# sabarim/STEm-Seg

Measured on AMD Instinct MI355X. Metric: clips/sec (T=8, 480p) embed+cluster, higher is better.
Workload: dtype f16x3: fp32 emulated from 2 fp16 terms per operand (22-bit operand significands; fp32 has 24), power-of-two operand scaling, 3 fp16 MFMA products per fp32 product, fp32 accumulate; |activation| >= 2.6e5 -> non-finite, flagged on the device, clip re-run in bf16x6

## Files before the change

stem-seg_amd/build.py:

```python
#!/usr/bin/env python3
import hashlib
import json
import os
import re
import subprocess
import sys
from concurrent.futures import ThreadPoolExecutor

HERE = os.path.dirname(os.path.abspath(__file__))
CSRC = os.path.join(HERE, "csrc")
LIBDIR = os.path.join(HERE, "stemseg_amd", "lib")
OBJDIR = os.path.join(CSRC, "build")
LIB = os.path.join(LIBDIR, "libstemseg_hip.so")
ARCH = "gfx950"
FLAGS = ["--offload-arch=" + ARCH, "-O3", "-std=c++17", "-fPIC", "-fno-gpu-rdc", "-Wall", "-Wno-unused-function"]
FLAGS += ["-Xclang", "-target-feature", "-Xclang", "-packed-fp32-ops"]
FLAGS += ["-save-temps=obj"]
PACKED_FP32 = re.compile(r"^\s+(v_pk_(?:fma|mul|add)_f32)\b")


def _sources():
    return sorted(f for f in os.listdir(CSRC) if f.endswith(".hip"))


def _digest():
    h = hashlib.sha256()
    h.update(" ".join(FLAGS).encode())
    for f in sorted(os.listdir(CSRC)) + [os.path.join("..", "..", "include", "stemseg_hip.h")]:
        p = os.path.join(CSRC, f)
        if os.path.isfile(p) and (f.endswith((".hip", ".h"))):
            h.update(f.encode())
            h.update(open(p, "rb").read())
    return h.hexdigest()


def isa_report():
    out = {}
    for src in _sources():
        path = os.path.join(OBJDIR, src.replace(".hip", "") + "-hip-amdgcn-amd-amdhsa-gfx950.s")
        kernels, by_kernel, cur = 0, {}, None
        if os.path.exists(path):
            for line in open(path, errors="replace"):
                m = re.match(r"^(_Z\w+|\w+):\s*(;.*)?$", line)
                if m and not line.startswith("."):
                    cur = m.group(1)
                if ".amdhsa_kernel " in line:
                    kernels += 1
                m = PACKED_FP32.match(line)
                if m and cur:
                    by_kernel[cur] = by_kernel.get(cur, 0) + 1
        out[src] = {"kernels": kernels, "packed_fp32_valu_instructions": sum(by_kernel.values()), "kernels_with_packed_fp32": len(by_kernel),
                    "assembly_found": os.path.exists(path)}
    return {"arch": ARCH, "no_packed_fp32_flag": True, "sources": out}


def build(force=False, verbose=True):
    os.makedirs(LIBDIR, exist_ok=True)
    os.makedirs(OBJDIR, exist_ok=True)
    stamp = os.path.join(OBJDIR, "libstemseg_hip.stamp")
    dig = _digest()
    if not force and os.path.exists(LIB) and os.path.exists(stamp) and open(stamp).read().strip() == dig:
        if verbose:
            print("[build] %s is up to date" % os.path.relpath(LIB, os.path.dirname(HERE)))
        return LIB
    hipcc = os.environ.get("HIPCC", "/opt/rocm/bin/hipcc")
    if not os.path.exists(hipcc):
        hipcc = "hipcc"

    def compile_one(src):
        obj = os.path.join(OBJDIR, src.replace(".hip", ".o"))
        cmd = [hipcc] + FLAGS + ["-c", os.path.join(CSRC, src), "-o", obj]
        r = subprocess.run(cmd, capture_output=True, text=True)
        if r.returncode != 0:
            raise RuntimeError("hipcc failed on %s:\n%s\n%s" % (src, r.stdout, r.stderr))
        err = "\n".join(l for l in r.stderr.splitlines() if "is not a recognized feature for this target" not in l).strip()
        if verbose and err:
            print(err)
        stem = os.path.join(OBJDIR, src.replace(".hip", ""))
        for ext in ("-hip-amdgcn-amd-amdhsa-gfx950.hipi", "-hip-amdgcn-amd-amdhsa-gfx950.bc", "-host-x86_64-unknown-linux-gnu.hipi",
                    "-host-x86_64-unknown-linux-gnu.bc", "-host-x86_64-unknown-linux-gnu.s"):
            if os.path.exists(stem + ext):
                os.remove(stem + ext)
        return obj

    with ThreadPoolExecutor(max_workers=min(8, os.cpu_count() or 2)) as ex:
# ... 21 lines not shown
```

stem-seg_amd/csrc/bottleneck_fused.hip:

```cpp
#include "common.h"
#include "split_operand.h"

namespace stemseg {

typedef float f32x16 __attribute__((ext_vector_type(16)));
typedef _Float16 f16x8 __attribute__((ext_vector_type(8)));
typedef unsigned int u32x4 __attribute__((ext_vector_type(4)));

struct FusedTailParams {
    const unsigned int* x16;
    const char* w3;
    const float* b3;
    const float* res;
    float* y;
    const char* w1;
    const float* b1;
    float* z;
    int64_t z_cs, z_ts, z_ys;
    int dec_H, dec_W;
    int V;
    const float* xs;
    const char* wd;
    const float* bd;
    float* xsub;
// ... 370 lines not shown

template <int MID_>
struct FusedTail16Cfg {
    static constexpr int MID = MID_, COUT = 4 * MID_, CT = 128;
    static constexpr int NW = 8, NTHREADS = 512, P = 16 * NW;
    static constexpr int NC3 = MID / 32, NCT = COUT / CT;
    static constexpr int NT3 = CT / 16, NT1 = MID / 16;
    static constexpr int SC = 2;
    static constexpr int NS = NC3 / SC, NU = CT / 32;
    static constexpr int W3_CHUNK = 8 * CT * 16;
    static constexpr int W3_BYTES = SC * W3_CHUNK;
    static constexpr int W1_BYTES = 8 * MID * 16;
    static constexpr int TAB_BYTES = 2 * CT * 4;
    static constexpr int LDS_BYTES = 2 * W3_BYTES + 2 * W1_BYTES + 2 * TAB_BYTES;
    static_assert(NC3 % SC == 0 && W3_BYTES % (1024 * NW) == 0 && W1_BYTES % (1024 * NW) == 0 && TAB_BYTES == 1024, "whole DMA pieces per wave");
    static_assert(W3_CHUNK == FT_WL.slab_bytes(CT, FT_WL.CK) && W1_BYTES == FT_WL.slab_bytes(MID, FT_WL.CK), "tile byte sizes follow the packed-weight layout");
    static_assert(LDS_BYTES <= 160 * 1024 && 2 * MID * 4 <= W3_BYTES, "LDS");
};

template <class C>
__global__ __launch_bounds__(C::NTHREADS, 2) void fused_tail16_kernel(const FusedTailParams p) {
#pragma clang fp contract(off)
    __shared__ __attribute__((aligned(1024))) char smem[C::LDS_BYTES];
    char* const w3buf = smem;
    char* const w1buf = smem + 2 * C::W3_BYTES;
    char* const tabbuf = smem + 2 * C::W3_BYTES + 2 * C::W1_BYTES;

    const int tid = threadIdx.x, lane = tid & 63;
    const int wave = __builtin_amdgcn_readfirstlane(tid >> 6);
    const int n = lane & 15, kb = lane >> 4;
    const int pos = blockIdx.x * C::P + wave * 16 + n;
    const bool pos_ok = pos < p.V;
    const int pos_c = min(pos, p.V - 1);
    const int64_t V = p.V;
    const unsigned int lane_off = (unsigned int)(((int64_t)(4 * kb) * V + pos_c) * 4);
    auto opaque = [](unsigned int v) __attribute__((always_inline)) { asm volatile("" : "+v"(v)); return v; };
    typedef const __attribute__((address_space(1))) void* gptr_t;
    typedef __attribute__((address_space(3))) void* lptr_t;
    const float* inv3 = reinterpret_cast<const float*>(p.w3 + FT_WL.inv_offset(C::COUT, C::MID));
    const float* inv1 = reinterpret_cast<const float*>(p.w1 + FT_WL.inv_offset(C::MID, C::COUT));

    auto dma_w3 = [&](const int j, const int st, const int buf) __attribute__((always_inline)) {
        constexpr int PER_ROW = C::CT * 16 / 1024, PER_CHUNK = C::W3_CHUNK / 1024;
#pragma unroll
        for (int k = 0; k < C::W3_BYTES / 1024 / C::NW; ++k) {
            const int idx = wave + k * C::NW, sc = idx / PER_CHUNK, r = idx % PER_CHUNK, row = r / PER_ROW, part = r % PER_ROW;
            const char* src = p.w3 + ((int64_t)(st * C::SC + sc) * 8 + row) * (C::COUT * 16) + (int64_t)j * (C::CT * 16) + part * 1024 + (size_t)(opaque((unsigned int)lane) * 16u);
            __builtin_amdgcn_global_load_lds((gptr_t)src, (lptr_t)(w3buf + buf * C::W3_BYTES + idx * 1024), 16, 0, 0);
        }
    };
    auto dma_w1 = [&](const int cc, const int buf) __attribute__((always_inline)) {
#pragma unroll
        for (int k = 0; k < C::W1_BYTES / 1024 / C::NW; ++k) {
            const int idx = wave + k * C::NW;
            const char* src = p.w1 + (int64_t)cc * C::W1_BYTES + (int64_t)idx * 1024 + (size_t)(opaque((unsigned int)lane) * 16u);
            __builtin_amdgcn_global_load_lds((gptr_t)src, (lptr_t)(w1buf + buf * C::W1_BYTES + idx * 1024), 16, 0, 0);
        }
    };
    auto dma_tab = [&](const int j) __attribute__((always_inline)) {
        if (wave == 0) {
            const unsigned int l = opaque((unsigned int)lane);
            const float* src = (l < 32 ? inv3 : p.b3 - C::CT) + (int64_t)j * C::CT + (size_t)(l * 4u);
            __builtin_amdgcn_global_load_lds((gptr_t)src, (lptr_t)(tabbuf + (j & 1) * C::TAB_BYTES), 16, 0, 0);
        }
    };
    auto dma_tail_tab = [&]() __attribute__((always_inline)) {
        constexpr int PIECES = (2 * C::MID + 255) / 256;
        if (wave < PIECES) {
            const unsigned int f0 = (unsigned int)wave * 256u + opaque((unsigned int)lane) * 4u;
            if (f0 < 2u * C::MID) {
                const float* src = (f0 < (unsigned int)C::MID ? inv1 : p.b1 - C::MID) + (size_t)f0;
                __builtin_amdgcn_global_load_lds((gptr_t)src, (lptr_t)(w3buf + wave * 1024), 16, 0, 0);
            }
        }
    };
    auto stage_sync = [&]() __attribute__((always_inline)) {
        __builtin_amdgcn_s_waitcnt(0x0f70);
        __syncthreads();
    };
    auto load_identity = [&](const int co_first, float (&rres)[8]) __attribute__((always_inline)) {
// ... 1 lines not shown
        for (int i = 0; i < 8; ++i)
            rres[i] = *reinterpret_cast<const float*>(reinterpret_cast<const char*>(p.res + (int64_t)(co_first + 16 * (i >> 2) + (i & 3)) * V) + (size_t)lane_off);
    };
    const f16x8 k2048 = {(_Float16)(1.0f / F16X3_LO_SCALE), (_Float16)(1.0f / F16X3_LO_SCALE), (_Float16)(1.0f / F16X3_LO_SCALE), (_Float16)(1.0f / F16X3_LO_SCALE),
                         (_Float16)(1.0f / F16X3_LO_SCALE), (_Float16)(1.0f / F16X3_LO_SCALE), (_Float16)(1.0f / F16X3_LO_SCALE), (_Float16)(1.0f / F16X3_LO_SCALE)};
    auto mma3x2 = [&](f32x4& c0, f32x4& c1, const f16x8 a0_hi, const f16x8 a0_lo, const f16x8 a1_hi, const f16x8 a1_lo, const f16x8 b_hi, const f16x8 b_lo)
        __attribute__((always_inline)) {
        const f16x8 a0_his = a0_hi * k2048, a1_his = a1_hi * k2048;
        c0 = __builtin_amdgcn_mfma_f32_16x16x32_f16(a0_lo, b_hi, c0, 0, 0, 0);
        c1 = __builtin_amdgcn_mfma_f32_16x16x32_f16(a1_lo, b_hi, c1, 0, 0, 0);
        c0 = __builtin_amdgcn_mfma_f32_16x16x32_f16(a0_his, b_lo, c0, 0, 0, 0);
        c1 = __builtin_amdgcn_mfma_f32_16x16x32_f16(a1_his, b_lo, c1, 0, 0, 0);
        c0 = __builtin_amdgcn_mfma_f32_16x16x32_f16(a0_hi, b_hi, c0, 0, 0, 0);
        c1 = __builtin_amdgcn_mfma_f32_16x16x32_f16(a1_hi, b_hi, c1, 0, 0, 0);
    };

    dma_w3(0, 0, 0);
    f16x8 xh[C::NC3], xl[C::NC3];
    {
        const char* xs = reinterpret_cast<const char*>(p.x16) + (size_t)((unsigned int)pos_c * 16u);
#pragma unroll
        for (int s = 0; s < C::NC3; ++s) {
            xh[s] = *reinterpret_cast<const f16x8*>(xs + ((int64_t)(4 * s + kb)) * V * 16);
            xl[s] = *reinterpret_cast<const f16x8*>(xs + ((int64_t)(C::MID / 8 + 4 * s + kb)) * V * 16);
        }
    }
    f32x4 acc1[C::NT1];
#pragma unroll
    for (int m = 0; m < C::NT1; ++m) acc1[m] = f32x4{0.f, 0.f, 0.f, 0.f};
    stage_sync();
    int sb = 0, eb = 0;
#pragma unroll 1
    for (int j = 0; j < C::NCT; ++j) {
        f32x4 acc3[C::NT3];
#pragma unroll
        for (int t = 0; t < C::NT3; ++t) acc3[t] = f32x4{0.f, 0.f, 0.f, 0.f};
        const int co_j = j * C::CT;
        float rres[8];
#pragma unroll
        for (int st = 0; st < C::NS; ++st) {
            if (st + 1 < C::NS) dma_w3(j, st + 1, sb ^ 1);
            else { dma_w1(j * C::NU, eb); dma_tab(j); load_identity(co_j, rres); }
            const char* wb = w3buf + sb * C::W3_BYTES + (((kb >> 1) * 2 * 2 + (kb & 1)) * C::CT + n) * 16;
            constexpr int NSTEP = C::SC * C::NT3 / 2;
            f16x8 a_hi[2][2], a_lo[2][2];
            auto ld_a = [&](const int i, const int k) __attribute__((always_inline)) {
                const int sc = (2 * i) / C::NT3, t = (2 * i) % C::NT3;
#pragma unroll
                for (int e = 0; e < 2; ++e) {
                    a_hi[k][e] = *reinterpret_cast<const f16x8*>(wb + sc * C::W3_CHUNK + (0 * 2 * C::CT + (t + e) * 16) * 16);
                    a_lo[k][e] = *reinterpret_cast<const f16x8*>(wb + sc * C::W3_CHUNK + (1 * 2 * C::CT + (t + e) * 16) * 16);
                }
            };
            ld_a(0, 0);
#pragma unroll
            for (int i = 0; i < NSTEP; ++i) {
                if (i + 1 < NSTEP) ld_a(i + 1, (i + 1) & 1);
                __builtin_amdgcn_sched_barrier(0);
                const int t = (2 * i) % C::NT3, ch = st * C::SC + (2 * i) / C::NT3;
                mma3x2(acc3[t], acc3[t + 1], a_hi[i & 1][0], a_lo[i & 1][0], a_hi[i & 1][1], a_lo[i & 1][1], xh[ch], xl[ch]);
                __builtin_amdgcn_sched_barrier(0);
            }
            stage_sync();
            sb ^= 1;
        }
        const float* tab = reinterpret_cast<const float*>(tabbuf + (j & 1) * C::TAB_BYTES);
// ... 31 lines not shown
                    auto s16 = __builtin_amdgcn_permlane16_swap(s32[0], s32[1], false, false);
                    bw[pl][i] = s16[0];
                    bw[pl][2 + i] = s16[1];
                }
            const u32x4 bh = {bw[0][0], bw[0][1], bw[0][2], bw[0][3]}, bl = {bw[1][0], bw[1][1], bw[1][2], bw[1][3]};
            const f16x8 b_hi = __builtin_bit_cast(f16x8, bh), b_lo = __builtin_bit_cast(f16x8, bl);
            __builtin_amdgcn_sched_barrier(0);
            if (u + 1 < C::NU) { dma_w1(j * C::NU + u + 1, eb ^ 1); load_identity(co_j + 32 * (u + 1), rres); }
            else if (j + 1 < C::NCT) dma_w3(j + 1, 0, sb);
            else dma_tail_tab();
            __builtin_amdgcn_sched_barrier(0);
            const char* w1b = w1buf + eb * C::W1_BYTES + (((kb >> 1) * 2 * 2 + (kb & 1)) * C::MID + n) * 16;
            f16x8 a_hi[1][2], a_lo[1][2];
            auto ld_a1 = [&](const int i, const int k) __attribute__((always_inline)) {
#pragma unroll
                for (int e = 0; e < 2; ++e) {
                    a_hi[k][e] = *reinterpret_cast<const f16x8*>(w1b + (0 * 2 * C::MID + (2 * i + e) * 16) * 16);
                    a_lo[k][e] = *reinterpret_cast<const f16x8*>(w1b + (1 * 2 * C::MID + (2 * i + e) * 16) * 16);
                }
            };
#pragma unroll
            for (int i = 0; i < C::NT1 / 2; ++i) {
                ld_a1(i, 0);
                __builtin_amdgcn_sched_barrier(0);
                mma3x2(acc1[2 * i], acc1[2 * i + 1], a_hi[0][0], a_lo[0][0], a_hi[0][1], a_lo[0][1], b_hi, b_lo);
                __builtin_amdgcn_sched_barrier(0);
            }
            stage_sync();
            eb ^= 1;
        }
    }
    if (pos_ok) {
        const int hwp = p.dec_H * p.dec_W;
        const int t2 = pos / hwp, r2 = pos - t2 * hwp, y2 = r2 / p.dec_W, x2 = r2 - y2 * p.dec_W;
        const unsigned int z_off = (unsigned int)(((int64_t)(4 * kb) * p.z_cs + (int64_t)t2 * p.z_ts + (int64_t)y2 * p.z_ys + x2) * 4);
        const float* ttab = reinterpret_cast<const float*>(w3buf);
#pragma unroll
        for (int m1 = 0; m1 < C::NT1; ++m1) {
            const int co4 = m1 * 16 + 4 * kb;
            const float4 sc = *reinterpret_cast<const float4*>(ttab + co4);
            const float4 bv = *reinterpret_cast<const float4*>(ttab + C::MID + co4);
            char* zo = reinterpret_cast<char*>(p.z + (int64_t)(m1 * 16) * p.z_cs);
            *reinterpret_cast<float*>(zo + (size_t)z_off) = relu_keep_nan(__fadd_rn(__fmul_rn(acc1[m1][0], sc.x), bv.x));
            *reinterpret_cast<float*>(zo + p.z_cs * 4 + (size_t)z_off) = relu_keep_nan(__fadd_rn(__fmul_rn(acc1[m1][1], sc.y), bv.y));
            *reinterpret_cast<float*>(zo + p.z_cs * 8 + (size_t)z_off) = relu_keep_nan(__fadd_rn(__fmul_rn(acc1[m1][2], sc.z), bv.z));
            *reinterpret_cast<float*>(zo + p.z_cs * 12 + (size_t)z_off) = relu_keep_nan(__fadd_rn(__fmul_rn(acc1[m1][3], sc.w), bv.w));
        }
    }
}


typedef __amdgpu_buffer_rsrc_t ft_rsrc_t;
#define FT_VMCNT_(n) __builtin_amdgcn_s_waitcnt(((n) & 15) | (((n) >> 4) << 14) | 0x0F70)
#define FT_VMCNT(n) FT_VMCNT_(n)
#define FT_SGB(mask, n) __builtin_amdgcn_sched_group_barrier(mask, n, 0)

template <int MID_, int CT_, int DS_ = 0, int N1_ = MID_, bool LAT_ = false>
struct FusedTailR1Cfg {
    static constexpr int MID = MID_, CT = CT_, COUT = 4 * MID_;
    static constexpr int N1 = N1_;
    static constexpr bool LAT = LAT_;
    static constexpr int EST = LAT ? 32 : 16;
    static constexpr int DS = DS_, NGD = DS_ / 16;
    static constexpr int NW = 4, NTHREADS = 64 * NW, P = 32 * NW;
    static constexpr int NC3 = MID / 32, NG = MID / 16, NCT = COUT / CT;
    static constexpr int MI3 = CT / 32, MI1 = N1 / 32;
    static constexpr int SC = 2;
    static constexpr int NS = NC3 / SC, NU = CT / 32;
    static constexpr int NSD = DS / 32 / SC;
    static_assert(DS % (32 * SC) == 0, "shortcut: whole stages");
    static constexpr int NX3 = SC * 2 * (MI3 / 2), NX1 = 2 * (MI1 / 2);
    static constexpr int W3_CHUNK = 8 * CT * 16, W3_BYTES = SC * W3_CHUNK;
    static constexpr int W1_BYTES = 8 * N1 * 16;
    static_assert(W3_CHUNK == FT_WL.slab_bytes(CT, FT_WL.CK) && W1_BYTES == FT_WL.slab_bytes(N1, FT_WL.CK), "tile byte sizes follow the packed-weight layout");
    static constexpr int TAB_BYTES = 1024;
    static constexpr int LDS_BYTES = 2 * W3_BYTES + 2 * W1_BYTES + 2 * TAB_BYTES;
    static constexpr int W3_PIECES = W3_BYTES / 1024 / NW, W1_PIECES = W1_BYTES / 1024 / NW;
    static constexpr int SL = 8 / NX1, S0 = NX1 / 4, M_PPS = 8 / S0;
    static_assert(NC3 % SC == 0 && MI3 % 2 == 0 && MI1 % 2 == 0 && W3_BYTES % (1024 * NW) == 0 && W1_BYTES % (1024 * NW) == 0 && 2 * CT * 4 <= TAB_BYTES, "whole DMA pieces per wave");
    static_assert(LDS_BYTES <= 160 * 1024 && 2 * N1 * 4 <= W3_BYTES && 16 + EST <= 63 && (NX1 == 8 || NX1 == 4) && NX3 == 8 && MI3 == 4 && NS >= 2 && NU >= 2 && NU % 2 == 0, "LDS / slice placement / identity buffer parity");
    static_assert(W3_PIECES == 8 && W1_PIECES <= 8, "the pieces of a stage are requested in its first steps");
    static_assert(NG * 8 + MI1 * 16 <= 256, "the conv3 input and conv1's accumulators are the AGPR half of the register file");
};

template <class C>
__global__ __launch_bounds__(C::NTHREADS, 1) void fused_tail_r1_kernel(const FusedTailParams p) {
#pragma clang fp contract(off)
    __shared__ __attribute__((aligned(1024))) char smem[C::LDS_BYTES];
    char* const w3buf = smem;
    char* const w1buf = smem + 2 * C::W3_BYTES;
    char* const tabbuf = smem + 2 * C::W3_BYTES + 2 * C::W1_BYTES;

    const int tid = threadIdx.x, lane = tid & 63;
    const int wave = __builtin_amdgcn_readfirstlane(tid >> 6);
    const int half = lane >> 5, l31 = lane & 31;
    const int pos = blockIdx.x * C::P + wave * 32 + l31;
    const bool pos_ok = pos < p.V;
    const int pos_c = min(pos, p.V - 1);
    const int64_t V = p.V;
    const unsigned int V4 = (unsigned int)p.V * 4u;
    const unsigned int lane_ld = (unsigned int)(4 * half) * V4 + (unsigned int)pos_c * 4u;
    const unsigned int lane_st = pos_ok ? lane_ld : 0xFFFFFF00u;
    const unsigned int tile_bytes = (unsigned int)C::CT * V4;
    const unsigned int SV4 = C::LAT ? (unsigned int)p.sub_V * 4u : 0u;
    unsigned int lane_sub = 0xFFFFFF00u;
    if constexpr (C::LAT) {
        const int hwp = p.dec_H * p.dec_W, t2 = pos_c / hwp, r2 = pos_c - t2 * hwp, y2 = r2 / p.dec_W, x2 = r2 - y2 * p.dec_W;
        if (pos_ok && !((y2 | x2) & 1)) lane_sub = (unsigned int)(4 * half) * SV4 + (unsigned int)((t2 * (p.dec_H / 2) + y2 / 2) * (p.dec_W / 2) + x2 / 2) * 4u;
    }
    typedef __attribute__((address_space(3))) void* lptr_t;
    const float* inv3 = reinterpret_cast<const float*>(p.w3 + FT_WL.inv_offset(C::COUT, C::MID));
    const float* inv1 = reinterpret_cast<const float*>(p.w1 + FT_WL.inv_offset(C::N1, C::COUT));

    const unsigned int lane16 = (unsigned int)lane * 16u;
    const unsigned int lds_w3 = (unsigned int)(uintptr_t)(lptr_t)w3buf, lds_w1 = (unsigned int)(uintptr_t)(lptr_t)w1buf;
    auto dma_piece = [&](const char* sbase, const unsigned int lds_addr) __attribute__((always_inline)) {
        asm volatile("s_mov_b32 m0, %0\n\ts_nop 0\n\tglobal_load_lds_dwordx4 %1, %2" : : "s"(lds_addr), "v"(lane16), "s"(sbase) : "memory");
    };
    auto dma_w3 = [&](const int j, const int st, const int buf, const int k) __attribute__((always_inline)) {
        constexpr int PER_ROW = C::CT * 16 / 1024, PER_CHUNK = C::W3_CHUNK / 1024;
        const int idx = wave + k * C::NW, sc = idx / PER_CHUNK, r = idx % PER_CHUNK, row = r / PER_ROW, part = r % PER_ROW;
        dma_piece(p.w3 + ((int64_t)(st * C::SC + sc) * 8 + row) * (C::COUT * 16) + (int64_t)j * (C::CT * 16) + part * 1024, lds_w3 + buf * C::W3_BYTES + idx * 1024);
    };
    auto dma_wd = [&](const int j, const int st, const int buf, const int k) __attribute__((always_inline)) {
        constexpr int PER_ROW = C::CT * 16 / 1024, PER_CHUNK = C::W3_CHUNK / 1024;
        const int idx = wave + k * C::NW, sc = idx / PER_CHUNK, r = idx % PER_CHUNK, row = r / PER_ROW, part = r % PER_ROW;
        dma_piece(p.wd + ((int64_t)(st * C::SC + sc) * 8 + row) * (C::COUT * 16) + (int64_t)j * (C::CT * 16) + part * 1024, lds_w3 + buf * C::W3_BYTES + idx * 1024);
    };
    auto dma_w1 = [&](const int cc, const int buf, const int k) __attribute__((always_inline)) {
        const int idx = wave + k * C::NW;
        dma_piece(p.w1 + (int64_t)cc * C::W1_BYTES + (int64_t)idx * 1024, lds_w1 + buf * C::W1_BYTES + idx * 1024);
    };
    float4 tabv = {0.f, 0.f, 0.f, 0.f};
    auto tab_fetch = [&](const int j) __attribute__((always_inline)) {
        if (wave == 0 && lane < 2 * (C::CT / 4))
            tabv = *reinterpret_cast<const float4*>((lane < C::CT / 4 ? inv3 : p.b3 - C::CT) + (int64_t)j * C::CT + lane * 4);
    };
    auto tab_store = [&](const int j) __attribute__((always_inline)) {
        if (wave == 0 && lane < 2 * (C::CT / 4)) *reinterpret_cast<float4*>(tabbuf + (j & 1) * C::TAB_BYTES + lane * 16) = tabv;
    };
    constexpr bool DSV = C::DS > 0;
    float4 tabdv = {0.f, 0.f, 0.f, 0.f};
    auto tabd_fetch = [&](const int j) __attribute__((always_inline)) {
        const float* invd = reinterpret_cast<const float*>(p.wd + FT_WL.inv_offset(C::COUT, C::DS));
        if (wave == 0 && lane < 2 * (C::CT / 4))
            tabdv = *reinterpret_cast<const float4*>((lane < C::CT / 4 ? invd : p.bd - C::CT) + (int64_t)j * C::CT + lane * 4);
    };
    auto tabd_store = [&](const int j) __attribute__((always_inline)) {
        if (wave == 0 && lane < 2 * (C::CT / 4)) *reinterpret_cast<float4*>(tabbuf + ((j + 1) & 1) * C::TAB_BYTES + lane * 16) = tabdv;
    };
    auto rsrc_of = [&](const float* base, const int jj) __attribute__((always_inline)) {
        return __builtin_amdgcn_make_buffer_rsrc(const_cast<float*>(base + (int64_t)jj * C::CT * V), 0, (int)tile_bytes, 0x00020000);
    };
    auto load_identity = [&](const int jj, const int u, float (&rr)[16]) __attribute__((always_inline)) {
        const ft_rsrc_t rs = rsrc_of(p.res, jj);
#pragma unroll
        for (int r = 0; r < 16; ++r)
            rr[r] = __builtin_bit_cast(float, __builtin_amdgcn_raw_buffer_load_b32(rs, lane_ld, (unsigned int)(32 * u + (r & 3) + 8 * (r >> 2)) * V4, 0));
    };
    const f16x8 k2048 = {(_Float16)(1.0f / F16X3_LO_SCALE), (_Float16)(1.0f / F16X3_LO_SCALE), (_Float16)(1.0f / F16X3_LO_SCALE), (_Float16)(1.0f / F16X3_LO_SCALE),
                         (_Float16)(1.0f / F16X3_LO_SCALE), (_Float16)(1.0f / F16X3_LO_SCALE), (_Float16)(1.0f / F16X3_LO_SCALE), (_Float16)(1.0f / F16X3_LO_SCALE)};
    auto mma6 = [&](f32x16& c0, f32x16& c1, const f16x8 (&a_hi)[2], const f16x8 (&a_lo)[2], const f16x8 (&a_his)[2], const f16x8 b_hi, const f16x8 b_lo)
        __attribute__((always_inline)) {
        c0 = __builtin_amdgcn_mfma_f32_32x32x16_f16(a_lo[0], b_hi, c0, 0, 0, 0);
        c1 = __builtin_amdgcn_mfma_f32_32x32x16_f16(a_lo[1], b_hi, c1, 0, 0, 0);
        c0 = __builtin_amdgcn_mfma_f32_32x32x16_f16(a_his[0], b_lo, c0, 0, 0, 0);
        c1 = __builtin_amdgcn_mfma_f32_32x32x16_f16(a_his[1], b_lo, c1, 0, 0, 0);
        c0 = __builtin_amdgcn_mfma_f32_32x32x16_f16(a_hi[0], b_hi, c0, 0, 0, 0);
        c1 = __builtin_amdgcn_mfma_f32_32x32x16_f16(a_hi[1], b_hi, c1, 0, 0, 0);
    };

#pragma unroll
    for (int k = 0; k < C::W3_PIECES; ++k) {
        if constexpr (DSV) dma_wd(0, 0, 0, k);
        else dma_w3(0, 0, 0, k);
    }
    float rres[2][16];
    if constexpr (!DSV) {
        load_identity(0, 0, rres[0]);
        load_identity(0, 1, rres[1]);
    }
    f16x8 xh[C::NG], xl[C::NG];
    {
        const char* xs = reinterpret_cast<const char*>(p.x16) + (size_t)((unsigned int)pos_c * 16u);
#pragma unroll
        for (int G = 0; G < C::NG; ++G) {
            xh[G] = *reinterpret_cast<const f16x8*>(xs + ((int64_t)(2 * G + half)) * V * 16);
            xl[G] = *reinterpret_cast<const f16x8*>(xs + ((int64_t)(C::MID / 8 + 2 * G + half)) * V * 16);
        }
    }
    f16x8 xdh[DSV ? C::NGD : 1], xdl[DSV ? C::NGD : 1];
    if constexpr (DSV) {
        const ft_rsrc_t rx = __builtin_amdgcn_make_buffer_rsrc(const_cast<float*>(p.xs), 0, (int)((unsigned int)C::DS * V4), 0x00020000);
        const unsigned int lane_xs = (unsigned int)(8 * half) * V4 + (unsigned int)pos_c * 4u;
#pragma unroll
        for (int G = 0; G < C::NGD; ++G) {
            float xr[8];
#pragma unroll
            for (int i = 0; i < 8; ++i) xr[i] = __builtin_bit_cast(float, __builtin_amdgcn_raw_buffer_load_b32(rx, lane_xs, (unsigned int)(16 * G + i) * V4, 0));
            u32x4 hw4, lw4;
#pragma unroll
            for (int i = 0; i < 4; ++i) {
                unsigned int hwd, lwd;
                split_pair_f16(xr[2 * i], xr[2 * i + 1], hwd, lwd);
                hw4[i] = hwd; lw4[i] = lwd;
            }
            xdh[G] = __builtin_bit_cast(f16x8, hw4);
            xdl[G] = __builtin_bit_cast(f16x8, lw4);
        }
    }
    f32x16 acc1[C::MI1];
#pragma unroll
    for (int m = 0; m < C::MI1; ++m)
#pragma unroll
        for (int r = 0; r < 16; ++r) acc1[m][r] = 0.f;
    FT_VMCNT(0);
    __syncthreads();
    int sb = 0, eb = 0;
#pragma unroll 1
    for (int j = 0; j < C::NCT; ++j) {
        f32x16 accd[DSV ? C::MI3 : 1];
        if constexpr (DSV) {
#pragma unroll
            for (int m = 0; m < C::MI3; ++m)
#pragma unroll
                for (int r = 0; r < 16; ++r) accd[m][r] = 0.f;
#pragma unroll
            for (int st = 0; st < C::NSD; ++st) {
                if (st == 0) tabd_fetch(j);
                const char* wb = w3buf + sb * C::W3_BYTES + (half * C::CT + l31) * 16;
                f16x8 a_hi[3][2], a_lo[3][2], a_his[2][2];
                auto ld3 = [&](const int s, const int k) __attribute__((always_inline)) {
                    const int mp = s / (2 * C::SC), sc = (s % (2 * C::SC)) / 2, g = s % 2;
#pragma unroll
                    for (int e = 0; e < 2; ++e) {
                        a_hi[k][e] = *reinterpret_cast<const f16x8*>(wb + sc * C::W3_CHUNK + (((g * 2 + 0) * 2) * C::CT + (2 * mp + e) * 32) * 16);
                        a_lo[k][e] = *reinterpret_cast<const f16x8*>(wb + sc * C::W3_CHUNK + (((g * 2 + 1) * 2) * C::CT + (2 * mp + e) * 32) * 16);
                    }
                };
                ld3(0, 0);
                ld3(1, 1);
                a_his[0][0] = a_hi[0][0] * k2048;
                a_his[0][1] = a_hi[0][1] * k2048;
#pragma unroll
                for (int s = 0; s < C::NX3; ++s) {
                    __builtin_amdgcn_sched_barrier(0);
                    if (s < 2) {
#pragma unroll
                        for (int k = 4 * s; k < 4 * s + 4; ++k) {
                            if (st + 1 < C::NSD) dma_wd(j, st + 1, sb ^ 1, k);
                            else dma_w3(j, 0, sb ^ 1, k);
                        }
                    }
                    if (s + 2 < C::NX3) ld3(s + 2, (s + 2) % 3);
                    if (s + 1 < C::NX3) {
                        a_his[(s + 1) & 1][0] = a_hi[(s + 1) % 3][0] * k2048;
                        a_his[(s + 1) & 1][1] = a_hi[(s + 1) % 3][1] * k2048;
                    }
                    const int mp = s / (2 * C::SC), sc = (s % (2 * C::SC)) / 2, g = s % 2, G = 2 * (st * C::SC + sc) + g;
                    mma6(accd[2 * mp], accd[2 * mp + 1], a_hi[s % 3], a_lo[s % 3], a_his[s & 1], xdh[G], xdl[G]);
#pragma unroll
                    for (int i = 0; i < 6; ++i) { FT_SGB(0x008, 1); FT_SGB(0x100, 1); FT_SGB(0x002, 2); }
                }
                __builtin_amdgcn_sched_barrier(0);
                FT_VMCNT(0);
                if (st == 0) tabd_store(j);
                __syncthreads();
                sb ^= 1;
            }
            const float* tabd = reinterpret_cast<const float*>(tabbuf + ((j + 1) & 1) * C::TAB_BYTES) + 4 * half;
#pragma unroll
            for (int u = 0; u < C::MI3; ++u)
#pragma unroll
                for (int q4 = 0; q4 < 4; ++q4) {
                    const float4 sc = *reinterpret_cast<const float4*>(tabd + 32 * u + 8 * q4);
                    const float4 bv = *reinterpret_cast<const float4*>(tabd + C::CT + 32 * u + 8 * q4);
                    accd[u][4 * q4 + 0] = __fadd_rn(__fmul_rn(accd[u][4 * q4 + 0], sc.x), bv.x);
                    accd[u][4 * q4 + 1] = __fadd_rn(__fmul_rn(accd[u][4 * q4 + 1], sc.y), bv.y);
                    accd[u][4 * q4 + 2] = __fadd_rn(__fmul_rn(accd[u][4 * q4 + 2], sc.z), bv.z);
                    accd[u][4 * q4 + 3] = __fadd_rn(__fmul_rn(accd[u][4 * q4 + 3], sc.w), bv.w);
                }
#pragma unroll
            for (int u = 0; u < C::MI3; ++u) asm volatile("" : "+v"(accd[u]));
            __builtin_amdgcn_sched_barrier(0);
        }
        f32x16 acc3[C::MI3];
#pragma unroll
        for (int m = 0; m < C::MI3; ++m)
#pragma unroll
            for (int r = 0; r < 16; ++r) acc3[m][r] = 0.f;
        const float* tab = reinterpret_cast<const float*>(tabbuf + (j & 1) * C::TAB_BYTES) + 4 * half;
        const ft_rsrc_t ry = rsrc_of(p.y, j);
        const ft_rsrc_t rsub = __builtin_amdgcn_make_buffer_rsrc(C::LAT ? p.xsub + (int64_t)j * C::CT * p.sub_V : p.y, 0, (int)((unsigned int)C::CT * SV4), 0x00020000);
        unsigned int hw[8], lw[8];
        f16x8 b_hi[2][2], b_lo[2][2];
        auto e_slice = [&](const int u, const int q4) __attribute__((always_inline)) {
            const int c4 = 32 * u + 8 * q4;
            const float4 sc = *reinterpret_cast<const float4*>(tab + c4);
            const float4 bv = *reinterpret_cast<const float4*>(tab + C::CT + c4);
            float rr[4];
#pragma unroll
            for (int i = 0; i < 4; ++i) rr[i] = DSV ? accd[DSV ? u : 0][4 * q4 + i] : rres[u & 1][4 * q4 + i];
            float v0 = __fmul_rn(acc3[u][4 * q4 + 0], sc.x), v1 = __fmul_rn(acc3[u][4 * q4 + 1], sc.y), v2 = __fmul_rn(acc3[u][4 * q4 + 2], sc.z),
                  v3 = __fmul_rn(acc3[u][4 * q4 + 3], sc.w);
            v0 = relu_keep_nan(__fadd_rn(__fadd_rn(v0, bv.x), rr[0]));
            v1 = relu_keep_nan(__fadd_rn(__fadd_rn(v1, bv.y), rr[1]));
            v2 = relu_keep_nan(__fadd_rn(__fadd_rn(v2, bv.z), rr[2]));
            v3 = relu_keep_nan(__fadd_rn(__fadd_rn(v3, bv.w), rr[3]));
            __builtin_amdgcn_raw_buffer_store_b32(__builtin_bit_cast(unsigned int, v0), ry, lane_st, (unsigned int)(c4 + 0) * V4, 0);
            __builtin_amdgcn_raw_buffer_store_b32(__builtin_bit_cast(unsigned int, v1), ry, lane_st, (unsigned int)(c4 + 1) * V4, 0);
            __builtin_amdgcn_raw_buffer_store_b32(__builtin_bit_cast(unsigned int, v2), ry, lane_st, (unsigned int)(c4 + 2) * V4, 0);
            __builtin_amdgcn_raw_buffer_store_b32(__builtin_bit_cast(unsigned int, v3), ry, lane_st, (unsigned int)(c4 + 3) * V4, 0);
            if constexpr (C::LAT) {
                __builtin_amdgcn_raw_buffer_store_b32(__builtin_bit_cast(unsigned int, v0), rsub, lane_sub, (unsigned int)(c4 + 0) * SV4, 0);
                __builtin_amdgcn_raw_buffer_store_b32(__builtin_bit_cast(unsigned int, v1), rsub, lane_sub, (unsigned int)(c4 + 1) * SV4, 0);
                __builtin_amdgcn_raw_buffer_store_b32(__builtin_bit_cast(unsigned int, v2), rsub, lane_sub, (unsigned int)(c4 + 2) * SV4, 0);
                __builtin_amdgcn_raw_buffer_store_b32(__builtin_bit_cast(unsigned int, v3), rsub, lane_sub, (unsigned int)(c4 + 3) * SV4, 0);
            }
            split_pair_f16(v0, v1, hw[2 * q4], lw[2 * q4]);
            split_pair_f16(v2, v3, hw[2 * q4 + 1], lw[2 * q4 + 1]);
        };
        auto e_perm = [&](const int gg, f16x8& bh, f16x8& bl) __attribute__((always_inline)) {
            unsigned int xh_[2], yh_[2], xl_[2], yl_[2];
#pragma unroll
            for (int i = 0; i < 2; ++i) {
                auto sh = __builtin_amdgcn_permlane32_swap(hw[4 * gg + i], hw[4 * gg + 2 + i], false, false);
                xh_[i] = sh[0]; yh_[i] = sh[1];
                auto sl = __builtin_amdgcn_permlane32_swap(lw[4 * gg + i], lw[4 * gg + 2 + i], false, false);
                xl_[i] = sl[0]; yl_[i] = sl[1];
            }
            const u32x4 bh4 = {xh_[0], xh_[1], yh_[0], yh_[1]}, bl4 = {xl_[0], xl_[1], yl_[0], yl_[1]};
            bh = __builtin_bit_cast(f16x8, bh4);
            bl = __builtin_bit_cast(f16x8, bl4);
        };
#pragma unroll
        for (int st = 0; st < C::NS; ++st) {
            if (st + 2 == C::NS) tab_fetch(j);
            const char* wb = w3buf + sb * C::W3_BYTES + (half * C::CT + l31) * 16;
            f16x8 a_hi[3][2], a_lo[3][2], a_his[2][2];
            auto ld3 = [&](const int s, const int k) __attribute__((always_inline)) {
                const int mp = s / (2 * C::SC), sc = (s % (2 * C::SC)) / 2, g = s % 2;
#pragma unroll
                for (int e = 0; e < 2; ++e) {
                    a_hi[k][e] = *reinterpret_cast<const f16x8*>(wb + sc * C::W3_CHUNK + (((g * 2 + 0) * 2) * C::CT + (2 * mp + e) * 32) * 16);
                    a_lo[k][e] = *reinterpret_cast<const f16x8*>(wb + sc * C::W3_CHUNK + (((g * 2 + 1) * 2) * C::CT + (2 * mp + e) * 32) * 16);
                }
            };
            ld3(0, 0);
            ld3(1, 1);
            a_his[0][0] = a_hi[0][0] * k2048;
            a_his[0][1] = a_hi[0][1] * k2048;
#pragma unroll
            for (int s = 0; s < C::NX3; ++s) {
                __builtin_amdgcn_sched_barrier(0);
                if (s < 2) {
#pragma unroll
                    for (int k = 4 * s; k < 4 * s + 4; ++k) {
                        if (st + 1 < C::NS) dma_w3(j, st + 1, sb ^ 1, k);
                        else if (k < C::W1_PIECES) dma_w1(j * C::NU, eb, k);
                    }
                }
                if (s + 2 < C::NX3) ld3(s + 2, (s + 2) % 3);
                if (s + 1 < C::NX3) {
                    a_his[(s + 1) & 1][0] = a_hi[(s + 1) % 3][0] * k2048;
                    a_his[(s + 1) & 1][1] = a_hi[(s + 1) % 3][1] * k2048;
                }
                if (st + 1 == C::NS && s >= C::NX3 / 2) e_slice(0, s - C::NX3 / 2);
                const int mp = s / (2 * C::SC), sc = (s % (2 * C::SC)) / 2, g = s % 2, G = 2 * (st * C::SC + sc) + g;
                mma6(acc3[2 * mp], acc3[2 * mp + 1], a_hi[s % 3], a_lo[s % 3], a_his[s & 1], xh[G], xl[G]);
#pragma unroll
                for (int i = 0; i < 6; ++i) {
                    FT_SGB(0x008, 1); FT_SGB(0x100, 1);
                    if (st + 1 == C::NS && s >= C::NX3 / 2) { FT_SGB(0x002, 7); FT_SGB(0x040, C::LAT ? 2 : 1); }
                    else FT_SGB(0x002, 2);
                }
            }
            __builtin_amdgcn_sched_barrier(0);
            if (st + 1 == C::NS) FT_VMCNT(C::EST);
            else FT_VMCNT(0);
            if (st + 2 == C::NS) tab_store(j);
            __syncthreads();
            sb ^= 1;
        }
        e_perm(0, b_hi[0][0], b_lo[0][0]);
        e_perm(1, b_hi[0][1], b_lo[0][1]);
#pragma unroll
        for (int u = 0; u < C::NU; ++u) {
            const char* w1b = w1buf + eb * C::W1_BYTES + (half * C::N1 + l31) * 16;
            f16x8 a_hi[3][2], a_lo[3][2], a_his[2][2];
            auto ld1 = [&](const int s, const int k) __attribute__((always_inline)) {
                const int g = s / (C::MI1 / 2), mp = s % (C::MI1 / 2);
#pragma unroll
                for (int e = 0; e < 2; ++e) {
                    a_hi[k][e] = *reinterpret_cast<const f16x8*>(w1b + (((g * 2 + 0) * 2) * C::N1 + (2 * mp + e) * 32) * 16);
                    a_lo[k][e] = *reinterpret_cast<const f16x8*>(w1b + (((g * 2 + 1) * 2) * C::N1 + (2 * mp + e) * 32) * 16);
                }
            };
            ld1(0, 0);
            ld1(1, 1);
            a_his[0][0] = a_hi[0][0] * k2048;
            a_his[0][1] = a_hi[0][1] * k2048;
#pragma unroll
            for (int s = 0; s < C::NX1; ++s) {
                __builtin_amdgcn_sched_barrier(0);
                if (s < C::S0) {
#pragma unroll
                    for (int k = C::M_PPS * s; k < C::M_PPS * s + C::M_PPS; ++k) {
                        if (u + 1 < C::NU) { if (k < C::W1_PIECES) dma_w1(j * C::NU + u + 1, eb ^ 1, k); }
                        else if (j + 1 < C::NCT) { if constexpr (DSV) dma_wd(j + 1, 0, sb, k); else dma_w3(j + 1, 0, sb, k); }
                    }
                }
                if (!DSV && s == C::S0) load_identity(u + 2 < C::NU ? j : min(j + 1, C::NCT - 1), (u + 2) % C::NU, rres[u & 1]);
                if (s + 2 < C::NX1) ld1(s + 2, (s + 2) % 3);
                if (s + 1 < C::NX1) {
                    a_his[(s + 1) & 1][0] = a_hi[(s + 1) % 3][0] * k2048;
                    a_his[(s + 1) & 1][1] = a_hi[(s + 1) % 3][1] * k2048;
                }
                if (u + 1 < C::NU) {
                    constexpr int SE = C::S0 + 4 / C::SL;
                    if (s >= C::S0 && s < SE) {
#pragma unroll
                        for (int q = 0; q < C::SL; ++q) e_slice(u + 1, (s - C::S0) * C::SL + q);
                    }
                    if (C::SL == 1 ? s == SE : s == SE) e_perm(0, b_hi[(u + 1) & 1][0], b_lo[(u + 1) & 1][0]);
                    if (C::SL == 1 ? s == SE + 1 : s == SE) e_perm(1, b_hi[(u + 1) & 1][1], b_lo[(u + 1) & 1][1]);
                }
                const int g = s / (C::MI1 / 2), mp = s % (C::MI1 / 2);
                mma6(acc1[2 * mp], acc1[2 * mp + 1], a_hi[s % 3], a_lo[s % 3], a_his[s & 1], b_hi[u & 1][g], b_lo[u & 1][g]);
#pragma unroll
                for (int i = 0; i < 6; ++i) { FT_SGB(0x008, 1); FT_SGB(0x100, 1); FT_SGB(0x002, 7 * C::SL); FT_SGB(0x040, C::SL * (C::LAT ? 2 : 1)); FT_SGB(0x020, 3); }
            }
            __builtin_amdgcn_sched_barrier(0);
            if (u + 1 < C::NU) FT_VMCNT(DSV ? C::EST : 16 + C::EST);
            else FT_VMCNT(DSV ? 0 : 16);
            __syncthreads();
            eb ^= 1;
        }
    }
    static_assert(C::N1 / 4 <= 64, "one lane per four channels");
    if (wave < 2 && lane < C::N1 / 4)
        *reinterpret_cast<float4*>(w3buf + wave * (C::N1 * 4) + lane * 16) = *reinterpret_cast<const float4*>((wave == 0 ? inv1 : p.b1) + lane * 4);
    __syncthreads();
    if (pos_ok) {
        const int hwp = p.dec_H * p.dec_W;
        const int t2 = pos / hwp, r2 = pos - t2 * hwp, y2 = r2 / p.dec_W, x2 = r2 - y2 * p.dec_W;
        const unsigned int z_off = (unsigned int)(((int64_t)(4 * half) * p.z_cs + (int64_t)t2 * p.z_ts + (int64_t)y2 * p.z_ys + x2) * 4);
        const float* ttab = reinterpret_cast<const float*>(w3buf);
#pragma unroll
        for (int m1 = 0; m1 < C::MI1; ++m1)
#pragma unroll
            for (int q = 0; q < 4; ++q) {
                const int co4 = m1 * 32 + 8 * q + 4 * half;
                const float4 sc = *reinterpret_cast<const float4*>(ttab + co4);
                const float4 bv = *reinterpret_cast<const float4*>(ttab + C::N1 + co4);
                char* zo = reinterpret_cast<char*>(p.z + (int64_t)(m1 * 32 + 8 * q) * p.z_cs);
                *reinterpret_cast<float*>(zo + (size_t)z_off) = slot_act<C::LAT>(__fadd_rn(__fmul_rn(acc1[m1][4 * q + 0], sc.x), bv.x));
                *reinterpret_cast<float*>(zo + p.z_cs * 4 + (size_t)z_off) = slot_act<C::LAT>(__fadd_rn(__fmul_rn(acc1[m1][4 * q + 1], sc.y), bv.y));
                *reinterpret_cast<float*>(zo + p.z_cs * 8 + (size_t)z_off) = slot_act<C::LAT>(__fadd_rn(__fmul_rn(acc1[m1][4 * q + 2], sc.z), bv.z));
                *reinterpret_cast<float*>(zo + p.z_cs * 12 + (size_t)z_off) = slot_act<C::LAT>(__fadd_rn(__fmul_rn(acc1[m1][4 * q + 3], sc.w), bv.w));
            }
    }
}

template <class C>
static int launch_fused_r1_cfg(const FusedTailParams& p, hipStream_t s) {
    const double flops = 2.0 * 2.0 * (double)C::MID * C::COUT * (double)p.V;
    void* ev = profile_begin(19, flops, s);
    hipLaunchKernelGGL(fused_tail_r1_kernel<C>, dim3((unsigned)ceil_div(p.V, C::P)), dim3(C::NTHREADS), 0, s, p);
    profile_end(ev, s);
    SS_LAUNCH_CHECK();
// ... 97 lines not shown
```

Measured before the change: 129.9.

## Strength-reduce DMA addressing and pin loop-invariant values in scalar registers

Reworks the weight-tile DMA address computation so each wave handles whole rows, using per-wave base pointers plus immediate LDS offsets through s_add into m0. Per-tile base pointers for weights, residual, output and subsample are advanced incrementally instead of being recomputed from j each iteration. Asm barriers pin V, V4 and SV4 to SGPRs and keep the accumulators in AGPRs, which is meant to avoid register spills and readlane/writelane traffic inside the MFMA loop. The build script also reports scratch size and lane-move counts per kernel. The risk is subtle addressing bugs in the new row-to-LDS mapping.

```diff
diff --git a/stem-seg_amd/build.py b/stem-seg_amd/build.py
--- a/stem-seg_amd/build.py
+++ b/stem-seg_amd/build.py
@@ -38,19 +38,35 @@
     out = {}
     for src in _sources():
         path = os.path.join(OBJDIR, src.replace(".hip", "") + "-hip-amdgcn-amd-amdhsa-gfx950.s")
-        kernels, by_kernel, cur = 0, {}, None
+        kernels, pk_by_kernel, cur = 0, {}, None
+        body, scratch = {}, {}
         if os.path.exists(path):
             for line in open(path, errors="replace"):
                 m = re.match(r"^(_Z\w+|\w+):\s*(;.*)?$", line)
                 if m and not line.startswith("."):
                     cur = m.group(1)
-                if ".amdhsa_kernel " in line:
+                    body[cur] = []
+                m = re.match(r"^\s+\.amdhsa_kernel\s+(\S+)", line)
+                if m:
                     kernels += 1
+                    cur = m.group(1)
+                m = re.match(r"^\s+\.amdhsa_private_segment_fixed_size\s+(\d+)", line)
+                if m and cur:
+                    scratch[cur] = int(m.group(1))
                 m = PACKED_FP32.match(line)
                 if m and cur:
-                    by_kernel[cur] = by_kernel.get(cur, 0) + 1
-        out[src] = {"kernels": kernels, "packed_fp32_valu_instructions": sum(by_kernel.values()), "kernels_with_packed_fp32": len(by_kernel),
-                    "assembly_found": os.path.exists(path)}
+                    pk_by_kernel[cur] = pk_by_kernel.get(cur, 0) + 1
+                m = re.match(r"^\s+([a-z][a-z0-9_]*)\b", line)
+                if m and cur in body:
+                    body[cur].append(m.group(1))
+        by_kernel = {}
+        for k, sc in scratch.items():
+            ops = body.get(k, [])
+            mf = [i for i, o in enumerate(ops) if o.startswith("v_mfma")]
+            loop = ops[mf[0]:mf[-1] + 1] if mf else []
+            by_kernel[k] = {"scratch": sc, "mfma": len(mf), "lane_moves_in_mfma_loop": sum(o in ("v_readlane_b32", "v_writelane_b32") for o in loop)}
+        out[src] = {"kernels": kernels, "packed_fp32_valu_instructions": sum(pk_by_kernel.values()), "kernels_with_packed_fp32": len(pk_by_kernel),
+                    "assembly_found": os.path.exists(path), "by_kernel": by_kernel}
     return {"arch": ARCH, "no_packed_fp32_flag": True, "sources": out}
 
 
diff --git a/stem-seg_amd/csrc/bottleneck_fused.hip b/stem-seg_amd/csrc/bottleneck_fused.hip
--- a/stem-seg_amd/csrc/bottleneck_fused.hip
+++ b/stem-seg_amd/csrc/bottleneck_fused.hip
@@ -426,7 +426,7 @@
     const int pos = blockIdx.x * C::P + wave * 16 + n;
     const bool pos_ok = pos < p.V;
     const int pos_c = min(pos, p.V - 1);
-    const int64_t V = p.V;
+    int64_t V = p.V;
     const unsigned int lane_off = (unsigned int)(((int64_t)(4 * kb) * V + pos_c) * 4);
     auto opaque = [](unsigned int v) __attribute__((always_inline)) { asm volatile("" : "+v"(v)); return v; };
     typedef const __attribute__((address_space(1))) void* gptr_t;
@@ -435,11 +435,12 @@
     const float* inv1 = reinterpret_cast<const float*>(p.w1 + FT_WL.inv_offset(C::MID, C::COUT));
 
     auto dma_w3 = [&](const int j, const int st, const int buf) __attribute__((always_inline)) {
-        constexpr int PER_ROW = C::CT * 16 / 1024, PER_CHUNK = C::W3_CHUNK / 1024;
+        constexpr int PER_ROW = C::CT * 16 / 1024;
+        static_assert((C::SC * 8) % C::NW == 0 && (C::W3_BYTES / 1024 / C::NW) % PER_ROW == 0, "a wave takes whole rows of a stage");
 #pragma unroll
         for (int k = 0; k < C::W3_BYTES / 1024 / C::NW; ++k) {
-            const int idx = wave + k * C::NW, sc = idx / PER_CHUNK, r = idx % PER_CHUNK, row = r / PER_ROW, part = r % PER_ROW;
-            const char* src = p.w3 + ((int64_t)(st * C::SC + sc) * 8 + row) * (C::COUT * 16) + (int64_t)j * (C::CT * 16) + part * 1024 + (size_t)(opaque((unsigned int)lane) * 16u);
+            const int q = k / PER_ROW, part = k % PER_ROW, row = wave + q * C::NW, idx = row * PER_ROW + part;
+            const char* src = p.w3 + ((int64_t)(st * C::SC) * 8 + row) * (C::COUT * 16) + (int64_t)j * (C::CT * 16) + part * 1024 + (size_t)(opaque((unsigned int)lane) * 16u);
             __builtin_amdgcn_global_load_lds((gptr_t)src, (lptr_t)(w3buf + buf * C::W3_BYTES + idx * 1024), 16, 0, 0);
         }
     };
@@ -507,6 +508,7 @@
     int sb = 0, eb = 0;
 #pragma unroll 1
     for (int j = 0; j < C::NCT; ++j) {
+        asm volatile("" : "+s"(V));
         f32x4 acc3[C::NT3];
 #pragma unroll
         for (int t = 0; t < C::NT3; ++t) acc3[t] = f32x4{0.f, 0.f, 0.f, 0.f};
@@ -604,7 +606,8 @@
     }
     if (pos_ok) {
         const int hwp = p.dec_H * p.dec_W;
-        const int t2 = pos / hwp, r2 = pos - t2 * hwp, y2 = r2 / p.dec_W, x2 = r2 - y2 * p.dec_W;
+        const int pos_e = blockIdx.x * C::P + wave * 16 + (int)(__builtin_amdgcn_mbcnt_hi(~0u, __builtin_amdgcn_mbcnt_lo(~0u, 0u)) & 15u);
+        const int t2 = pos_e / hwp, r2 = pos_e - t2 * hwp, y2 = r2 / p.dec_W, x2 = r2 - y2 * p.dec_W;
         const unsigned int z_off = (unsigned int)(((int64_t)(4 * kb) * p.z_cs + (int64_t)t2 * p.z_ts + (int64_t)y2 * p.z_ys + x2) * 4);
         const float* ttab = reinterpret_cast<const float*>(w3buf);
 #pragma unroll
@@ -670,11 +673,11 @@
     const bool pos_ok = pos < p.V;
     const int pos_c = min(pos, p.V - 1);
     const int64_t V = p.V;
-    const unsigned int V4 = (unsigned int)p.V * 4u;
+    unsigned int V4 = (unsigned int)p.V * 4u;
     const unsigned int lane_ld = (unsigned int)(4 * half) * V4 + (unsigned int)pos_c * 4u;
     const unsigned int lane_st = pos_ok ? lane_ld : 0xFFFFFF00u;
     const unsigned int tile_bytes = (unsigned int)C::CT * V4;
-    const unsigned int SV4 = C::LAT ? (unsigned int)p.sub_V * 4u : 0u;
+    unsigned int SV4 = C::LAT ? (unsigned int)p.sub_V * 4u : 0u;
     unsigned int lane_sub = 0xFFFFFF00u;
     if constexpr (C::LAT) {
         const int hwp = p.dec_H * p.dec_W, t2 = pos_c / hwp, r2 = pos_c - t2 * hwp, y2 = r2 / p.dec_W, x2 = r2 - y2 * p.dec_W;
@@ -685,47 +688,48 @@
     const float* inv1 = reinterpret_cast<const float*>(p.w1 + FT_WL.inv_offset(C::N1, C::COUT));
 
     const unsigned int lane16 = (unsigned int)lane * 16u;
-    const unsigned int lds_w3 = (unsigned int)(uintptr_t)(lptr_t)w3buf, lds_w1 = (unsigned int)(uintptr_t)(lptr_t)w1buf;
-    auto dma_piece = [&](const char* sbase, const unsigned int lds_addr) __attribute__((always_inline)) {
-        asm volatile("s_mov_b32 m0, %0\n\ts_nop 0\n\tglobal_load_lds_dwordx4 %1, %2" : : "s"(lds_addr), "v"(lane16), "s"(sbase) : "memory");
-    };
-    auto dma_w3 = [&](const int j, const int st, const int buf, const int k) __attribute__((always_inline)) {
-        constexpr int PER_ROW = C::CT * 16 / 1024, PER_CHUNK = C::W3_CHUNK / 1024;
-        const int idx = wave + k * C::NW, sc = idx / PER_CHUNK, r = idx % PER_CHUNK, row = r / PER_ROW, part = r % PER_ROW;
-        dma_piece(p.w3 + ((int64_t)(st * C::SC + sc) * 8 + row) * (C::COUT * 16) + (int64_t)j * (C::CT * 16) + part * 1024, lds_w3 + buf * C::W3_BYTES + idx * 1024);
-    };
-    auto dma_wd = [&](const int j, const int st, const int buf, const int k) __attribute__((always_inline)) {
-        constexpr int PER_ROW = C::CT * 16 / 1024, PER_CHUNK = C::W3_CHUNK / 1024;
-        const int idx = wave + k * C::NW, sc = idx / PER_CHUNK, r = idx % PER_CHUNK, row = r / PER_ROW, part = r % PER_ROW;
-        dma_piece(p.wd + ((int64_t)(st * C::SC + sc) * 8 + row) * (C::COUT * 16) + (int64_t)j * (C::CT * 16) + part * 1024, lds_w3 + buf * C::W3_BYTES + idx * 1024);
-    };
-    auto dma_w1 = [&](const int cc, const int buf, const int k) __attribute__((always_inline)) {
-        const int idx = wave + k * C::NW;
-        dma_piece(p.w1 + (int64_t)cc * C::W1_BYTES + (int64_t)idx * 1024, lds_w1 + buf * C::W1_BYTES + idx * 1024);
-    };
+    constexpr int PER_ROW = C::CT * 16 / 1024, ROW_STRIDE = C::COUT * 16;
+    static_assert((C::SC * 8) % C::NW == 0 && C::W3_PIECES == PER_ROW * (C::SC * 8 / C::NW), "a wave takes whole rows of a stage");
+    const unsigned int lds_w3w = (unsigned int)(uintptr_t)(lptr_t)w3buf + (unsigned int)wave * (PER_ROW * 1024);
+    const unsigned int lds_w1w = (unsigned int)(uintptr_t)(lptr_t)w1buf + (unsigned int)wave * 1024;
+    const char* w3w = p.w3 + (int64_t)wave * ROW_STRIDE;
+    const char* wdw = C::DS > 0 ? p.wd + (int64_t)wave * ROW_STRIDE : nullptr;
+    const char* w1w = p.w1 + (int64_t)wave * 1024;
+    auto dma_piece = [&](const char* src, const unsigned int lds_base, const int lds_off) __attribute__((always_inline)) {
+        asm volatile("s_add_u32 m0, %0, %1\n\ts_nop 0\n\tglobal_load_lds_dwordx4 %2, %3" : : "s"(lds_base), "i"(lds_off), "v"(lane16), "s"(src) : "memory", "scc");
+    };
+    auto dma_wc = [&](const char* wj, const int dj, const int st, const int buf, const int k) __attribute__((always_inline)) {
+        const int q = k / PER_ROW, part = k % PER_ROW;
+        dma_piece(wj + ((int64_t)(st * C::SC * 8 + C::NW * q) * ROW_STRIDE + dj * (C::CT * 16) + part * 1024), lds_w3w + buf * C::W3_BYTES, (C::NW * q * PER_ROW + part) * 1024);
+    };
+    auto dma_w1 = [&](const char* wj, const int u, const int buf, const int k) __attribute__((always_inline)) {
+        dma_piece(wj + ((int64_t)u * C::W1_BYTES + k * (C::NW * 1024)), lds_w1w + buf * C::W1_BYTES, k * (C::NW * 1024));
+    };
+    constexpr bool TAB_ALL = 2 * (C::CT / 4) >= 64;
+    auto tab_wave = [&]() __attribute__((always_inline)) { int w = wave; asm volatile("" : "+s"(w)); return w == 0; };
     float4 tabv = {0.f, 0.f, 0.f, 0.f};
     auto tab_fetch = [&](const int j) __attribute__((always_inline)) {
-        if (wave == 0 && lane < 2 * (C::CT / 4))
+        if (tab_wave() && (TAB_ALL || lane < 2 * (C::CT / 4)))
             tabv = *reinterpret_cast<const float4*>((lane < C::CT / 4 ? inv3 : p.b3 - C::CT) + (int64_t)j * C::CT + lane * 4);
     };
     auto tab_store = [&](const int j) __attribute__((always_inline)) {
-        if (wave == 0 && lane < 2 * (C::CT / 4)) *reinterpret_cast<float4*>(tabbuf + (j & 1) * C::TAB_BYTES + lane * 16) = tabv;
+        if (tab_wave() && (TAB_ALL || lane < 2 * (C::CT / 4))) *reinterpret_cast<float4*>(tabbuf + (j & 1) * C::TAB_BYTES + lane * 16) = tabv;
     };
     constexpr bool DSV = C::DS > 0;
     float4 tabdv = {0.f, 0.f, 0.f, 0.f};
     auto tabd_fetch = [&](const int j) __attribute__((always_inline)) {
         const float* invd = reinterpret_cast<const float*>(p.wd + FT_WL.inv_offset(C::COUT, C::DS));
-        if (wave == 0 && lane < 2 * (C::CT / 4))
+        if (tab_wave() && (TAB_ALL || lane < 2 * (C::CT / 4)))
             tabdv = *reinterpret_cast<const float4*>((lane < C::CT / 4 ? invd : p.bd - C::CT) + (int64_t)j * C::CT + lane * 4);
     };
     auto tabd_store = [&](const int j) __attribute__((always_inline)) {
-        if (wave == 0 && lane < 2 * (C::CT / 4)) *reinterpret_cast<float4*>(tabbuf + ((j + 1) & 1) * C::TAB_BYTES + lane * 16) = tabdv;
-    };
-    auto rsrc_of = [&](const float* base, const int jj) __attribute__((always_inline)) {
-        return __builtin_amdgcn_make_buffer_rsrc(const_cast<float*>(base + (int64_t)jj * C::CT * V), 0, (int)tile_bytes, 0x00020000);
-    };
-    auto load_identity = [&](const int jj, const int u, float (&rr)[16]) __attribute__((always_inline)) {
-        const ft_rsrc_t rs = rsrc_of(p.res, jj);
+        if (tab_wave() && (TAB_ALL || lane < 2 * (C::CT / 4))) *reinterpret_cast<float4*>(tabbuf + ((j + 1) & 1) * C::TAB_BYTES + lane * 16) = tabdv;
+    };
+    auto rsrc_at = [&](const char* rows) __attribute__((always_inline)) {
+        return __builtin_amdgcn_make_buffer_rsrc(const_cast<char*>(rows), 0, (int)tile_bytes, 0x00020000);
+    };
+    auto load_identity = [&](const char* rows, const int u, float (&rr)[16]) __attribute__((always_inline)) {
+        const ft_rsrc_t rs = rsrc_at(rows);
 #pragma unroll
         for (int r = 0; r < 16; ++r)
             rr[r] = __builtin_bit_cast(float, __builtin_amdgcn_raw_buffer_load_b32(rs, lane_ld, (unsigned int)(32 * u + (r & 3) + 8 * (r >> 2)) * V4, 0));
@@ -744,13 +748,13 @@
 
 #pragma unroll
     for (int k = 0; k < C::W3_PIECES; ++k) {
-        if constexpr (DSV) dma_wd(0, 0, 0, k);
-        else dma_w3(0, 0, 0, k);
+        if constexpr (DSV) dma_wc(wdw, 0, 0, 0, k);
+        else dma_wc(w3w, 0, 0, 0, k);
     }
     float rres[2][16];
     if constexpr (!DSV) {
-        load_identity(0, 0, rres[0]);
-        load_identity(0, 1, rres[1]);
+        load_identity(reinterpret_cast<const char*>(p.res), 0, rres[0]);
+        load_identity(reinterpret_cast<const char*>(p.res), 1, rres[1]);
     }
     f16x8 xh[C::NG], xl[C::NG];
     {
@@ -789,8 +793,15 @@
     FT_VMCNT(0);
     __syncthreads();
     int sb = 0, eb = 0;
+    const char *w3j = w3w, *wdj = wdw, *w1j = w1w;
+    const char* resj = reinterpret_cast<const char*>(p.res);
+    char* yj = reinterpret_cast<char*>(p.y);
+    char* subj = reinterpret_cast<char*>(C::LAT ? p.xsub : p.y);
 #pragma unroll 1
     for (int j = 0; j < C::NCT; ++j) {
+        asm volatile("" : "+s"(w3j), "+s"(w1j), "+s"(V4));
+        if constexpr (C::LAT) asm volatile("" : "+s"(SV4));
+        if constexpr (DSV) asm volatile("" : "+s"(wdj));
         f32x16 accd[DSV ? C::MI3 : 1];
         if constexpr (DSV) {
 #pragma unroll
@@ -820,8 +831,8 @@
                     if (s < 2) {
 #pragma unroll
                         for (int k = 4 * s; k < 4 * s + 4; ++k) {
-                            if (st + 1 < C::NSD) dma_wd(j, st + 1, sb ^ 1, k);
-                            else dma_w3(j, 0, sb ^ 1, k);
+                            if (st + 1 < C::NSD) dma_wc(wdj, 0, st + 1, sb ^ 1, k);
+                            else dma_wc(w3j, 0, 0, sb ^ 1, k);
                         }
                     }
                     if (s + 2 < C::NX3) ld3(s + 2, (s + 2) % 3);
@@ -862,8 +873,8 @@
 #pragma unroll
             for (int r = 0; r < 16; ++r) acc3[m][r] = 0.f;
         const float* tab = reinterpret_cast<const float*>(tabbuf + (j & 1) * C::TAB_BYTES) + 4 * half;
-        const ft_rsrc_t ry = rsrc_of(p.y, j);
-        const ft_rsrc_t rsub = __builtin_amdgcn_make_buffer_rsrc(C::LAT ? p.xsub + (int64_t)j * C::CT * p.sub_V : p.y, 0, (int)((unsigned int)C::CT * SV4), 0x00020000);
+        const ft_rsrc_t ry = rsrc_at(yj);
+        const ft_rsrc_t rsub = __builtin_amdgcn_make_buffer_rsrc(subj, 0, (int)((unsigned int)C::CT * SV4), 0x00020000);
         unsigned int hw[8], lw[8];
         f16x8 b_hi[2][2], b_lo[2][2];
         auto e_slice = [&](const int u, const int q4) __attribute__((always_inline)) {
@@ -928,8 +939,8 @@
                 if (s < 2) {
 #pragma unroll
                     for (int k = 4 * s; k < 4 * s + 4; ++k) {
-                        if (st + 1 < C::NS) dma_w3(j, st + 1, sb ^ 1, k);
-                        else if (k < C::W1_PIECES) dma_w1(j * C::NU, eb, k);
+                        if (st + 1 < C::NS) dma_wc(w3j, 0, st + 1, sb ^ 1, k);
+                        else if (k < C::W1_PIECES) dma_w1(w1j, 0, eb, k);
                     }
                 }
                 if (s + 2 < C::NX3) ld3(s + 2, (s + 2) % 3);
@@ -978,11 +989,11 @@
                 if (s < C::S0) {
 #pragma unroll
                     for (int k = C::M_PPS * s; k < C::M_PPS * s + C::M_PPS; ++k) {
-                        if (u + 1 < C::NU) { if (k < C::W1_PIECES) dma_w1(j * C::NU + u + 1, eb ^ 1, k); }
-                        else if (j + 1 < C::NCT) { if constexpr (DSV) dma_wd(j + 1, 0, sb, k); else dma_w3(j + 1, 0, sb, k); }
+                        if (u + 1 < C::NU) { if (k < C::W1_PIECES) dma_w1(w1j, u + 1, eb ^ 1, k); }
+                        else if (j + 1 < C::NCT) { if constexpr (DSV) dma_wc(wdj, 1, 0, sb, k); else dma_wc(w3j, 1, 0, sb, k); }
                     }
                 }
-                if (!DSV && s == C::S0) load_identity(u + 2 < C::NU ? j : min(j + 1, C::NCT - 1), (u + 2) % C::NU, rres[u & 1]);
+                if (!DSV && s == C::S0) load_identity(u + 2 < C::NU || j + 1 == C::NCT ? resj : resj + tile_bytes, (u + 2) % C::NU, rres[u & 1]);
                 if (s + 2 < C::NX1) ld1(s + 2, (s + 2) % 3);
                 if (s + 1 < C::NX1) {
                     a_his[(s + 1) & 1][0] = a_hi[(s + 1) % 3][0] * k2048;
@@ -1003,11 +1014,19 @@
                 for (int i = 0; i < 6; ++i) { FT_SGB(0x008, 1); FT_SGB(0x100, 1); FT_SGB(0x002, 7 * C::SL); FT_SGB(0x040, C::SL * (C::LAT ? 2 : 1)); FT_SGB(0x020, 3); }
             }
             __builtin_amdgcn_sched_barrier(0);
+#pragma unroll
+            for (int m = 0; m < C::MI1; ++m) asm volatile("" : "+a"(acc1[m]));
             if (u + 1 < C::NU) FT_VMCNT(DSV ? C::EST : 16 + C::EST);
             else FT_VMCNT(DSV ? 0 : 16);
             __syncthreads();
             eb ^= 1;
         }
+        w3j += C::CT * 16;
+        if constexpr (DSV) wdj += C::CT * 16;
+        w1j += (int64_t)C::NU * C::W1_BYTES;
+        if constexpr (!DSV) resj += tile_bytes;
+        yj += tile_bytes;
+        if constexpr (C::LAT) subj += (unsigned int)C::CT * SV4;
     }
     static_assert(C::N1 / 4 <= 64, "one lane per four channels");
     if (wave < 2 && lane < C::N1 / 4)
```

Result: no change. 130.7 (median of 6 runs) (+0.6%).
